# dusk-network/plonk_gadgets

Hardware: AMD Instinct MI355X
Metric: gadget constraints/sec (range_check 256-bit) (higher is better)
Workload: dtype u64x4 (BLS12-381 scalar, Montgomery limbs)

## Files before the change

### plonk_gadgets_amd/csrc/capi_composer.inc

```

struct pg_composer {
    pg_engine *e = nullptr;
    hipStream_t stream = nullptr;
    uint64_t gate_cap = 0, var_cap = 0, n = 0, nvars = 0, zero_var = 0;
    pg::ComposerCols cols{};
    uint64_t *d_stage = nullptr;
    std::vector<uint64_t> pi_gate;
    std::vector<pg_scalar> pi_val;
    std::vector<pg::FourthWire> fourth;
    std::vector<pg::PermSeg> segs;
    void *perm_small = nullptr, *perm_big = nullptr, *val_ws = nullptr;
    void *perm_pieces = nullptr;
    size_t perm_pieces_bytes = 0;
    size_t perm_small_bytes = 0, perm_big_bytes = 0, val_ws_bytes = 0;
    std::vector<void *> ragged;
    uint64_t *h_total = nullptr;
    uint64_t perm_last_sparse = 0;
    uint64_t sparse_hint = 0;
    uint64_t sparse_cap_first = 0;
    bool auto_grow = false;
    uint64_t col_stride = 0;
    void *block = nullptr;
    struct Queued {
        uint8_t kind;
// ... 1245 lines not shown
    add_ragged_segment(c, batch, lay.n_gates, lay.n_vars, 2 * 255 + 5, 255 + 262, b.row_off, b.var_off, 0, pg::WIRES_MAX_BOUND);
    c->n += lay.n_gates;
    c->nvars += lay.n_vars;
    return PG_OK;
}

pg_status pg_composer_is_non_zero_batch(pg_composer *c, const pg_variable *d_var, uint64_t batch, uint8_t *d_err_mask,
                                        uint64_t *err_count) {
    if (!c) return fail(PG_ERR_INVALID_ARGUMENT, "composer is NULL");
    PG_TRY(flush(c));
    if (err_count) *err_count = 0;
    if (batch == 0) return PG_OK;
    PG_TRY(check_u64s(d_var, "d_var"));
    pg_composer::Sig dg;
    PG_TRY(check_var_arrays(c, {d_var}, batch, &dg));
    PG_HIP_TRY(hipSetDevice(c->e->device));
    PG_TRY(perm_reserve(c, &c->val_ws, &c->val_ws_bytes, batch * 32));
    uint4 *vals = static_cast<uint4 *>(c->val_ws);
    const uint64_t want = (2 * batch + pg::kThreads - 1) / pg::kThreads;
    const uint32_t grid = (uint32_t)(want < (uint64_t)c->e->num_cus * 32 ? want : (uint64_t)c->e->num_cus * 32);
    hipLaunchKernelGGL(pg::gather_wire_values_kernel, dim3(grid), dim3(pg::kThreads), 0, c->stream, d_var, c->cols.vars, batch, vals);
    PG_HIP_TRY(hipGetLastError());
    RaggedBuffers b;
    PG_TRY(ragged_alloc(batch, false, &b));
    pg_layout lay;
    uint64_t errs = 0;
    pg_status st = pg_is_non_zero_plan(c->e, reinterpret_cast<const pg_scalar *>(vals), batch, b.row_off, b.var_off, d_err_mask, &lay,
                                       &errs, c->stream);
    const bool failed_items = st == PG_ERR_NON_EXISTING_INVERSE;
    if (failed_items) st = PG_OK;
    if (st == PG_OK) st = need(c, lay.n_gates, lay.n_vars);
    if (st == PG_OK) {
        const pg_columns at = cols_at(c, c->n, c->nvars);
        SignedAppend sa(c, gadget_sig(c, 28, pg::fr_zero(), pg::fr_zero(), batch, errs ? 0x8000000000000000ull | ++c->unmatched : 0, dg),
                        lay.n_gates);
        st = is_non_zero_common(c->e, d_var, reinterpret_cast<const pg_scalar *>(vals), batch, b.row_off, b.var_off, c->n, c->nvars,
                                c->zero_var, &at, c->stream, sa.in_place);
        if (st == PG_OK) sa.commit();
    }
    if (st != PG_OK) {
        (void)hipStreamSynchronize(c->stream);
        b.release();
        return st;
    }
    b.keep(c);
    if (errs == 0)
        add_segment(c, batch, lay.n_gates, lay.n_vars, 2, pg::WIRES_IS_NON_ZERO);
    else
        add_ragged_segment(c, batch, lay.n_gates, lay.n_vars, 3, 3, b.row_off, b.var_off, 2, pg::WIRES_IS_NON_ZERO);
    c->n += lay.n_gates;
    c->nvars += lay.n_vars;
    if (err_count) *err_count = errs;
    return failed_items ? fail(PG_ERR_NON_EXISTING_INVERSE, std::to_string(errs) + " item(s) without an inverse") : PG_OK;
}

pg_status pg_composer_scalar_mix_batch(pg_composer *c, const pg_scalar *d_v, const pg_scalar *d_y, const pg_scalar *d_s,
                                       const pg_scalar *d_a, const pg_scalar *d_b, uint64_t batch, pg_variable *d_result_vars,
                                       uint8_t *d_err_mask, uint64_t *err_count) {
    if (!c) return fail(PG_ERR_INVALID_ARGUMENT, "composer is NULL");
    PG_TRY(flush(c));
    if (err_count) *err_count = 0;
    if (batch == 0) return PG_OK;
    PG_HIP_TRY(hipSetDevice(c->e->device));
    RaggedBuffers b;
    PG_TRY(ragged_alloc(batch, false, &b));
    pg_layout lay;
    uint64_t errs = 0;
    pg_status st = pg_scalar_mix_plan(c->e, d_v, batch, b.row_off, b.var_off, d_err_mask, &lay, &errs, c->stream);
    const bool failed_items = st == PG_ERR_NON_EXISTING_INVERSE;
    if (failed_items) st = PG_OK;
    if (st == PG_OK) st = need(c, lay.n_gates, lay.n_vars);
    if (st == PG_OK) {
        const pg_columns at = cols_at(c, c->n, c->nvars);
        SignedAppend sa(c, gadget_sig(c, 13, pg::fr_zero(), pg::fr_zero(), batch, errs ? 0x8000000000000000ull | ++c->unmatched : 0), lay.n_gates);
        st = scalar_mix_common(c->e, d_v, d_y, d_s, d_a, d_b, batch, b.row_off, b.var_off, c->n, c->nvars, c->zero_var, &at, d_result_vars,
                               c->stream, sa.in_place);
        if (st == PG_OK) sa.commit();
    }
    if (st != PG_OK) {
        (void)hipStreamSynchronize(c->stream);
        b.release();
        return st;
    }
    b.keep(c);
    if (errs == 0)
        add_segment(c, batch, lay.n_gates, lay.n_vars, 0, pg::WIRES_MIX, 0);
    else
        add_ragged_segment(c, batch, lay.n_gates, lay.n_vars, 10, 15, b.row_off, b.var_off, 0, pg::WIRES_MIX);
    c->n += lay.n_gates;
    c->nvars += lay.n_vars;
    if (err_count) *err_count = errs;
    return failed_items ? fail(PG_ERR_NON_EXISTING_INVERSE, std::to_string(errs) + " item(s) without an inverse") : PG_OK;
}

namespace {
pg_status gate_batch(pg_composer *c, uint32_t op, const pg_variable *d_a, const pg_variable *d_b, const pg_variable *d_c,
                     const pg::Fr &q_m, const pg::Fr &q_l, const pg::Fr &q_r, const pg::Fr &q_o, const pg::Fr &q_c, uint64_t batch,
                     pg_variable *d_out_vars) {
    if (!c) return fail(PG_ERR_INVALID_ARGUMENT, "composer is NULL");
    PG_TRY(flush(c));
    if (batch == 0) return PG_OK;
    const bool creates = op == pg::OP_ADD || op == pg::OP_MUL;
    PG_TRY(check_u64s(d_a, "first Variable array"));
    PG_TRY(check_u64s(d_b, "second Variable array"));
    if (!creates) PG_TRY(check_u64s(d_c, "third Variable array"));
    PG_TRY(check_u64s(d_out_vars, "d_out_vars", true));
    for (const pg::Fr *q : {&q_m, &q_l, &q_r, &q_o, &q_c})
        if (!is_reduced(*q)) return fail(PG_ERR_INVALID_ARGUMENT, "selector is not a reduced BlsScalar");
    pg_composer::Sig dg;
    PG_TRY(check_var_arrays(c, {d_a, d_b == d_a ? nullptr : d_b, creates || d_c == d_a ? nullptr : d_c}, batch, &dg));
    PG_TRY(need(c, batch, creates ? batch : 0));
    PG_HIP_TRY(hipSetDevice(c->e->device));
    SigHasher h;
    h.u64(29); h.u64(op); h.u64(batch); h.u64((d_b == d_a ? 1 : 0) | (!creates && d_c == d_a ? 2 : 0) | (!creates && d_c == d_b ? 4 : 0));
    h.fr(q_m); h.fr(q_l); h.fr(q_r); h.fr(q_o); h.fr(q_c); h.u64(dg.a); h.u64(dg.b);
    h.u64(c->n); h.u64(c->nvars); h.u64(c->zero_var);
    SignedAppend sa(c, h.done(), batch);
    pg::GateBatch B{};
    B.op = op | (sa.in_place ? pg::OP_ROW_IN_PLACE : 0u); B.gate0 = c->n; B.var0 = c->nvars; B.batch = batch;
    B.a = d_a; B.b = d_b; B.c = creates ? nullptr : d_c; B.out_vars = d_out_vars;
    B.q_m = q_m; B.q_l = q_l; B.q_r = q_r; B.q_o = q_o; B.q_c = q_c;
    const uint64_t want = (batch + pg::kThreads - 1) / pg::kThreads, most = (uint64_t)c->e->num_cus * 32;
    hipLaunchKernelGGL(pg::gate_batch_kernel, dim3((uint32_t)(want < most ? want : most)), dim3(pg::kThreads), 0, c->stream, B, c->cols);
    PG_HIP_TRY(hipGetLastError());
    sa.commit();
    if (creates || batch >= 4096) add_segment(c, batch, batch, creates ? batch : 0, creates ? 2 : 3, creates ? pg::WIRES_GATE_OUT : pg::WIRES_GATE_ROWS);
    c->n += batch;
    if (creates) c->nvars += batch;
    return PG_OK;
}
}

pg_status pg_composer_poly_gate_batch(pg_composer *c, const pg_variable *d_a, const pg_variable *d_b, const pg_variable *d_c,
                                      const pg_scalar *q_m, const pg_scalar *q_l, const pg_scalar *q_r, const pg_scalar *q_o,
                                      const pg_scalar *q_c, uint64_t batch) {
    if (!q_m || !q_l || !q_r || !q_o || !q_c) return fail(PG_ERR_INVALID_ARGUMENT, "NULL argument");
    return gate_batch(c, pg::OP_ROW, d_a, d_b, d_c, to_fr(q_m), to_fr(q_l), to_fr(q_r), to_fr(q_o), to_fr(q_c), batch, nullptr);
}
pg_status pg_composer_add_batch(pg_composer *c, const pg_scalar *q_l, const pg_variable *d_a, const pg_scalar *q_r,
                                const pg_variable *d_b, const pg_scalar *q_c, uint64_t batch, pg_variable *d_out_vars) {
    if (!q_l || !q_r || !q_c) return fail(PG_ERR_INVALID_ARGUMENT, "NULL argument");
    return gate_batch(c, pg::OP_ADD, d_a, d_b, nullptr, pg::fr_zero(), to_fr(q_l), to_fr(q_r), pg::fr_neg_one(), to_fr(q_c), batch, d_out_vars);
}
pg_status pg_composer_mul_batch(pg_composer *c, const pg_scalar *q_m, const pg_variable *d_a, const pg_variable *d_b,
                                const pg_scalar *q_c, uint64_t batch, pg_variable *d_out_vars) {
    if (!q_m || !q_c) return fail(PG_ERR_INVALID_ARGUMENT, "NULL argument");
    return gate_batch(c, pg::OP_MUL, d_a, d_b, nullptr, to_fr(q_m), pg::fr_zero(), pg::fr_zero(), pg::fr_neg_one(), to_fr(q_c), batch, d_out_vars);
}
pg_status pg_composer_constrain_to_constant_batch(pg_composer *c, const pg_variable *d_a, const pg_scalar *constant, uint64_t batch) {
    if (!constant) return fail(PG_ERR_INVALID_ARGUMENT, "NULL argument");
    return gate_batch(c, pg::OP_ROW, d_a, d_a, d_a, pg::fr_zero(), pg::fr_one(), pg::fr_zero(), pg::fr_zero(), pg::fr_neg(to_fr(constant)),
                      batch, nullptr);
}
pg_status pg_composer_boolean_gate_batch(pg_composer *c, const pg_variable *d_a, uint64_t batch) {
    return gate_batch(c, pg::OP_ROW, d_a, d_a, d_a, pg::fr_one(), pg::fr_zero(), pg::fr_zero(), pg::fr_neg_one(), pg::fr_zero(), batch, nullptr);
}

pg_status pg_composer_add_input_batch(pg_composer *c, const pg_scalar *d_scalars, uint64_t batch, pg_variable *first_var) {
    if (!c || !first_var) return fail(PG_ERR_INVALID_ARGUMENT, "NULL argument");
    PG_TRY(flush(c));
    PG_TRY(need(c, 0, batch));
    if (batch) {
        PG_TRY(check_scalars(d_scalars, "d_scalars"));
        PG_HIP_TRY(hipSetDevice(c->e->device));
        PG_HIP_TRY(hipMemcpyAsync(c->cols.vars + 2 * c->nvars, d_scalars, batch * 32, hipMemcpyDeviceToDevice, c->stream));
    }
    *first_var = c->nvars;
    c->nvars += batch;
    return PG_OK;
}

pg_status pg_composer_copy_out(pg_composer *c, uint64_t gate_first, uint64_t n_gates, uint64_t var_first, uint64_t n_vars,
                               const pg_columns *dst) {
    if (!c || !dst) return fail(PG_ERR_INVALID_ARGUMENT, "NULL argument");
    PG_TRY(flush(c));
    if (gate_first + n_gates > c->n || var_first + n_vars > c->nvars) return fail(PG_ERR_INVALID_ARGUMENT, "range past the end");
    PG_HIP_TRY(hipSetDevice(c->e->device));
    const pg_columns src = cols_at(c, gate_first, var_first);
    pg_scalar *const ds[5] = {dst->q_m, dst->q_l, dst->q_r, dst->q_o, dst->q_c};
    const pg_scalar *const ss[5] = {src.q_m, src.q_l, src.q_r, src.q_o, src.q_c};
    for (int i = 0; i < 5; i++)
        if (ds[i] && n_gates) PG_HIP_TRY(hipMemcpyAsync(ds[i], ss[i], n_gates * 32, hipMemcpyDeviceToDevice, c->stream));
    uint64_t *const dw[3] = {dst->w_l, dst->w_r, dst->w_o};
    const uint64_t *const sw[3] = {src.w_l, src.w_r, src.w_o};
    for (int i = 0; i < 3; i++)
        if (dw[i] && n_gates) PG_HIP_TRY(hipMemcpyAsync(dw[i], sw[i], n_gates * 8, hipMemcpyDeviceToDevice, c->stream));
    if (dst->var_values && n_vars)
        PG_HIP_TRY(hipMemcpyAsync(dst->var_values, src.var_values, n_vars * 32, hipMemcpyDeviceToDevice, c->stream));
    return PG_OK;
}

pg_status pg_composer_read_value(pg_composer *c, pg_variable v, pg_scalar *out) {
    if (!c || !out) return fail(PG_ERR_INVALID_ARGUMENT, "NULL argument");
    PG_TRY(flush(c));
    PG_TRY(check_var(c, v));
    PG_HIP_TRY(hipMemcpyAsync(out, c->cols.vars + 2 * v, 32, hipMemcpyDeviceToHost, c->stream));
    PG_HIP_TRY(hipStreamSynchronize(c->stream));
    return PG_OK;
}

static pg_status upload_sparse(pg_composer *c, CallBuffers &B, uint64_t **d_gate, uint4 **d_val, pg::FourthWire **d_fw) {
    *d_gate = nullptr; *d_val = nullptr; *d_fw = nullptr;
    const size_t np = c->pi_gate.size(), nf = c->fourth.size();
    if (np) {
        PG_HIP_TRY(hipMalloc(d_gate, np * 8));
        B.own(*d_gate);
        PG_HIP_TRY(hipMalloc(d_val, np * 32));
        B.own(*d_val);
        PG_HIP_TRY(hipMemcpyAsync(*d_gate, c->pi_gate.data(), np * 8, hipMemcpyHostToDevice, c->stream));
        PG_HIP_TRY(hipMemcpyAsync(*d_val, c->pi_val.data(), np * 32, hipMemcpyHostToDevice, c->stream));
    }
    if (nf) {
        PG_HIP_TRY(hipMalloc(d_fw, nf * sizeof(pg::FourthWire)));
        B.own(*d_fw);
        PG_HIP_TRY(hipMemcpyAsync(*d_fw, c->fourth.data(), nf * sizeof(pg::FourthWire), hipMemcpyHostToDevice, c->stream));
    }
    return PG_OK;
}

pg_status pg_composer_check(pg_composer *c, int64_t *first_bad) {
    if (!c || !first_bad) return fail(PG_ERR_INVALID_ARGUMENT, "NULL argument");
    PG_TRY(flush(c));
    PG_HIP_TRY(hipSetDevice(c->e->device));
    CallBuffers B(c->stream);
    uint64_t *d_gate; uint4 *d_val; pg::FourthWire *d_fw;
    PG_TRY(upload_sparse(c, B, &d_gate, &d_val, &d_fw));
    unsigned long long *d_bad = nullptr, h_bad = ~0ull;
    PG_HIP_TRY(hipMalloc(&d_bad, 8));
    B.own(d_bad);
    PG_HIP_TRY(hipMemcpyAsync(d_bad, &h_bad, 8, hipMemcpyHostToDevice, c->stream));
    const uint64_t want = (c->n + pg::kThreads - 1) / pg::kThreads;
    const uint32_t grid = (uint32_t)(want < (uint64_t)c->e->num_cus * 8 ? (want ? want : 1) : (uint64_t)c->e->num_cus * 8);
    hipLaunchKernelGGL(pg::check_kernel, dim3(grid), dim3(pg::kThreads), 0, c->stream, c->cols, c->n, (uint64_t)0, c->nvars,
                       c->zero_var, d_gate, d_val, (uint32_t)c->pi_gate.size(), d_fw, (uint32_t)c->fourth.size(), d_bad);
    PG_HIP_TRY(hipGetLastError());
    PG_HIP_TRY(hipMemcpyAsync(&h_bad, d_bad, 8, hipMemcpyDeviceToHost, c->stream));
    PG_HIP_TRY(hipStreamSynchronize(c->stream));
    *first_bad = h_bad == ~0ull ? -1 : (int64_t)h_bad;
    return PG_OK;
}

pg_status pg_composer_dense_pi(pg_composer *c, pg_scalar *d_out) {
    if (!c) return fail(PG_ERR_INVALID_ARGUMENT, "composer is NULL");
    PG_TRY(flush(c));
    PG_TRY(check_scalars(d_out, "d_out"));
    PG_HIP_TRY(hipSetDevice(c->e->device));
    PG_HIP_TRY(hipMemsetAsync(d_out, 0, c->n * 32, c->stream));
    CallBuffers B(c->stream);
    uint64_t *d_gate; uint4 *d_val; pg::FourthWire *d_fw;
    PG_TRY(upload_sparse(c, B, &d_gate, &d_val, &d_fw));
    const uint32_t np = (uint32_t)c->pi_gate.size();
    if (np) {
        hipLaunchKernelGGL(pg::scatter_pi_kernel, dim3((np + 255) / 256), dim3(256), 0, c->stream,
                           reinterpret_cast<uint4 *>(d_out), d_gate, d_val, np);
        PG_HIP_TRY(hipGetLastError());
    }
    PG_HIP_TRY(hipStreamSynchronize(c->stream));
    return PG_OK;
}

pg_status pg_composer_materialize(pg_composer *c, const pg_full_columns *out) {
    if (!c || !out) return fail(PG_ERR_INVALID_ARGUMENT, "NULL argument");
    PG_TRY(flush(c));
    PG_HIP_TRY(hipSetDevice(c->e->device));
    const uint32_t grid = (uint32_t)c->e->num_cus * 32;
    pg::MaterializeOut M{};
    pg_scalar *const consts[7] = {out->q_4, out->q_arith, out->q_range, out->q_logic, out->q_fixed_group_add,
                                  out->q_variable_group_add, out->w_4_value};
    for (int k = 0; k < 7; k++) {
        if (!consts[k]) continue;
        PG_TRY(check_scalars(consts[k], "constant column"));
        M.konst[k] = reinterpret_cast<uint4 *>(consts[k]);
    }
    pg_scalar *const vals[3] = {out->w_l_value, out->w_r_value, out->w_o_value};
    for (int i = 0; i < 3; i++) {
        if (!vals[i]) continue;
        PG_TRY(check_scalars(vals[i], "wire value column"));
        M.val[i] = reinterpret_cast<uint4 *>(vals[i]);
    }
    if (out->w_4) {
        PG_TRY(check_u64s(out->w_4, "w_4"));
        M.w_4 = out->w_4;
    }
    const auto generic = [&](uint64_t lo, uint64_t hi) {
        if (hi <= lo) return;
        const uint64_t want = (2 * (hi - lo) + 16383) / 16384;
        hipLaunchKernelGGL(pg::materialize_kernel, dim3((uint32_t)(want < grid ? want : grid)), dim3(pg::kThreads), 0, c->stream, c->cols, M,
                           lo, hi, c->zero_var);
    };
    uint64_t at = 0;
    for (const pg::PermSeg &s : c->segs) {
        if (s.V > pg::kMatWindowVars || s.V == 0 || s.gate_end - s.gate_base < 4096) continue;
        generic(at, s.gate_base);
        uint64_t group = pg::kMatWindowVars / (s.V ? s.V : 1);
        group = group < 1 ? 1 : (group > s.items ? s.items : group);
#ifndef PG_MAT_GRID_PER_CU
#define PG_MAT_GRID_PER_CU 64
#endif
        const uint64_t n_groups = (s.items + group - 1) / group, most = (uint64_t)c->e->num_cus * PG_MAT_GRID_PER_CU;
        const dim3 mgrid((uint32_t)(n_groups < most ? n_groups : most));
        const bool closed = s.wire_kind != pg::WIRES_UNKNOWN && !s.row_off && (pg::ladder_foreign_per_item(s.wire_kind) == 0 || group <= pg::kMatWitItems);
#define PG_MAT_LAUNCH(MODE, KIND)                                                                                                          \
    hipLaunchKernelGGL((pg::materialize_items_kernel<MODE, KIND>), mgrid, dim3(pg::kMatThreads), 0, c->stream, c->cols, M, s, (uint32_t)group, \
                       c->zero_var)
        if (s.row_off && s.wire_kind == pg::WIRES_MAX_BOUND && group <= pg::kMatWitItems)
            hipLaunchKernelGGL((pg::materialize_items_kernel<pg::MAT_SELF, pg::WIRES_MAX_BOUND, true>), mgrid, dim3(pg::kMatThreads), 0, c->stream,
                               c->cols, M, s, (uint32_t)group, c->zero_var);
        else if (s.row_off && s.wire_kind == pg::WIRES_MIX && group < 127)
            hipLaunchKernelGGL((pg::materialize_items_kernel<pg::MAT_SELF, pg::WIRES_MIX, true>), mgrid, dim3(pg::kMatThreads), 0, c->stream,
                               c->cols, M, s, (uint32_t)group, c->zero_var);
        else if (!closed) PG_MAT_LAUNCH(pg::MAT_READ_WIRES, pg::WIRES_UNKNOWN);
        else if (s.wire_kind == pg::WIRES_RANGE_CHECK) PG_MAT_LAUNCH(pg::MAT_SELF, pg::WIRES_RANGE_CHECK);
        else if (s.wire_kind == pg::WIRES_MAX_BOUND) PG_MAT_LAUNCH(pg::MAT_SELF, pg::WIRES_MAX_BOUND);
        else if (s.wire_kind == pg::WIRES_RANGE_CHECK_ALLOCATED) PG_MAT_LAUNCH(pg::MAT_SELF, pg::WIRES_RANGE_CHECK_ALLOCATED);
        else if (s.wire_kind == pg::WIRES_MAX_BOUND_ALLOCATED) PG_MAT_LAUNCH(pg::MAT_SELF, pg::WIRES_MAX_BOUND_ALLOCATED);
        else if (s.wire_kind == pg::WIRES_DECOMPOSITION) PG_MAT_LAUNCH(pg::MAT_SELF, pg::WIRES_DECOMPOSITION);
        else if (s.wire_kind == pg::WIRES_MIX) PG_MAT_LAUNCH(pg::MAT_SELF, pg::WIRES_MIX);
        else PG_MAT_LAUNCH(pg::MAT_READ_WIRES, pg::WIRES_UNKNOWN);
#undef PG_MAT_LAUNCH
        at = s.gate_end;
    }
    generic(at, c->n);
    CallBuffers B(c->stream);
    uint64_t *d_gate; uint4 *d_val; pg::FourthWire *d_fw;
    PG_TRY(upload_sparse(c, B, &d_gate, &d_val, &d_fw));
    if (d_fw)
        hipLaunchKernelGGL(pg::patch_fourth_kernel, dim3(1), dim3(64), 0, c->stream, reinterpret_cast<uint4 *>(out->q_4), out->w_4,
                           reinterpret_cast<uint4 *>(out->w_4_value), c->cols.vars, d_fw, (uint32_t)c->fourth.size());
    PG_HIP_TRY(hipGetLastError());
    PG_HIP_TRY(hipStreamSynchronize(c->stream));
    return PG_OK;
}

#ifndef PG_PERM_LDS_PAD
#define PG_PERM_LDS_PAD 0
#endif
static pg_status perm_reserve(pg_composer *c, void **buf, size_t *have, size_t bytes) {
    if (bytes <= *have) return PG_OK;
    PG_HIP_TRY(hipStreamSynchronize(c->stream));
    if (*buf) (void)hipFree(*buf);
    *buf = nullptr;
    *have = 0;
    PG_HIP_TRY(hipMalloc(buf, bytes));
    *have = bytes;
    return PG_OK;
}

pg_status pg_composer_permutation_reserve(pg_composer *c, uint64_t sparse_positions) {
    if (!c) return fail(PG_ERR_INVALID_ARGUMENT, "composer is NULL");
    c->sparse_cap_first = sparse_positions;
    if (sparse_positions) c->perm_last_sparse = 0;
    return PG_OK;
}

pg_status pg_composer_permutation(pg_composer *c, uint64_t padded_n, uint64_t *d_sigma) {
    if (!c) return fail(PG_ERR_INVALID_ARGUMENT, "composer is NULL");
    PG_TRY(flush(c));
    PG_TRY(check_u64s(d_sigma, "d_sigma"));
    if (padded_n < c->n) return fail(PG_ERR_INVALID_ARGUMENT, "padded_n is smaller than the circuit");
    PG_HIP_TRY(hipSetDevice(c->e->device));
    const uint32_t grid = (uint32_t)c->e->num_cus * 32;
    if (!c->h_total) PG_HIP_TRY(hipHostMalloc(reinterpret_cast<void **>(&c->h_total), 32, hipHostMallocDefault));
    uint32_t pos_bits = 2, var_bits = 1;
    while ((1ull << pos_bits) < 4 * c->n) pos_bits++;
    while ((1ull << var_bits) < c->nvars + 1) var_bits++;
    if (pos_bits + var_bits > 64) return fail(PG_ERR_INVALID_ARGUMENT, "circuit too large for 64-bit (Variable, position) keys");
    std::vector<pg::PermSeg> segs;
    std::vector<std::pair<uint64_t, uint64_t>> gaps;
    uint64_t at = 0, gap_rows = 0;
    for (pg::PermSeg s : c->segs) {
        const auto fits = [&](uint64_t k) {
            return 4 * k * s.L < pg::kPermDone && k * s.V < pg::kPermNone &&
                   pg::perm_local_lds_bytes((uint32_t)(k * s.L), (uint32_t)(k * s.V)) <= pg::kPermLocalLdsLimit;
        };
        if (!fits(1)) continue;
        uint64_t k = 1024 / s.L;
        k = k < 1 ? 1 : (k > s.items ? s.items : k);
        while (k > 1 && !fits(k)) k--;
        const bool closed_ladder = s.wire_kind != pg::WIRES_UNKNOWN && s.wire_kind < pg::WIRES_MIX && (s.row_off ? s.wire_kind == pg::WIRES_MAX_BOUND && s.tail == 0 : s.wire_n >= 2);
        if (closed_ladder || (pg::is_template_kind(s.wire_kind) && s.tail == 0)) k = 1;
        s.group = (uint32_t)k;
        if (s.gate_base > at) gaps.emplace_back(at, s.gate_base);
        segs.push_back(s);
        at = s.gate_end;
    }
    if (c->n > at) gaps.emplace_back(at, c->n);
    for (const auto &g : gaps) gap_rows += g.second - g.first;
    const size_t seg_bytes = (segs.size() * sizeof(pg::PermSeg) + 255) / 256 * 256;
    const size_t fw_bytes = (c->fourth.size() * sizeof(pg::FourthWire) + 255) / 256 * 256;
    PG_TRY(perm_reserve(c, &c->perm_small, &c->perm_small_bytes, seg_bytes + fw_bytes + 256));
    char *small = static_cast<char *>(c->perm_small);
    pg::PermCtx X;
    X.C = c->cols; X.n = c->n; X.padded_n = padded_n; X.zero_var = c->zero_var;
    X.segs = reinterpret_cast<const pg::PermSeg *>(small); X.n_segs = (uint32_t)segs.size();
    X.fw = reinterpret_cast<const pg::FourthWire *>(small + seg_bytes); X.n_fw = (uint32_t)c->fourth.size();
    X.fw_lo = 0; X.fw_span = 0; X.pos_bits = pos_bits;
    X.hole_key = pos_bits + var_bits >= 64 ? ~0ull : (1ull << (pos_bits + var_bits)) - 1;
    if (!c->fourth.empty()) {
        uint64_t lo = ~0ull, hi = 0;
        for (const pg::FourthWire &f : c->fourth) { lo = f.gate < lo ? f.gate : lo; hi = f.gate > hi ? f.gate : hi; }
        X.fw_lo = lo; X.fw_span = hi - lo;
    }
    uint64_t reserved = 0;
    for (pg::PermSeg &s : segs)
        if (s.wire_kind != pg::WIRES_UNKNOWN && !s.row_off && s.wire_n >= 2) {
            s.sparse_base = reserved;
            reserved += s.items * pg::ladder_foreign_per_item(s.wire_kind);
        } else if (pg::is_template_kind(s.wire_kind) && s.tail == 0) {
            s.sparse_base = reserved;
            reserved += s.items * pg::template_foreign_per_item(s.wire_kind);
        }
    const auto ragged_ladder = [](const pg::PermSeg &s) { return s.row_off && s.wire_kind == pg::WIRES_MAX_BOUND && s.tail == 0; };
    const auto template_seg = [](const pg::PermSeg &s) { return pg::is_template_kind(s.wire_kind) && s.tail == 0; };
    const auto needs_pieces = [&](const pg::PermSeg &s) { return ragged_ladder(s) || (template_seg(s) && s.row_off); };
    const auto pieces_of = [](const pg::PermSeg &s) { return (s.gate_end - (s.gate_base & ~1ull) + pg::kPermLadderRows - 1) / pg::kPermLadderRows; };
    {
        uint64_t total_pieces = 0;
        for (const pg::PermSeg &s : segs)
            if (needs_pieces(s)) total_pieces += pieces_of(s);
        if (total_pieces) {
            PG_TRY(perm_reserve(c, &c->perm_pieces, &c->perm_pieces_bytes, total_pieces * sizeof(uint32_t)));
            uint32_t *at_piece = static_cast<uint32_t *>(c->perm_pieces);
            for (pg::PermSeg &s : segs)
                if (needs_pieces(s)) {
                    s.piece_item = at_piece;
                    at_piece += pieces_of(s);
                    const uint64_t want = (s.items + pg::kThreads - 1) / pg::kThreads;
                    hipLaunchKernelGGL(pg::perm_piece_items_kernel, dim3((uint32_t)(want < grid ? want : grid)), dim3(pg::kThreads), 0, c->stream, s,
                                       pg::kPermLadderRows, at_piece - pieces_of(s));
                }
            PG_HIP_TRY(hipGetLastError());
        }
    }
    unsigned long long *d_count = reinterpret_cast<unsigned long long *>(small + seg_bytes + fw_bytes);
    if (!segs.empty())
        PG_HIP_TRY(hipMemcpyAsync(small, segs.data(), segs.size() * sizeof(pg::PermSeg), hipMemcpyHostToDevice, c->stream));
    if (!c->fourth.empty())
        PG_HIP_TRY(hipMemcpyAsync(small + seg_bytes, c->fourth.data(), c->fourth.size() * sizeof(pg::FourthWire),
                                  hipMemcpyHostToDevice, c->stream));
    uint64_t cap = c->sparse_cap_first ? c->sparse_cap_first : 4 * gap_rows + c->sparse_hint + (1ull << 16), nS = 0;
    if (cap < c->perm_last_sparse) cap = c->perm_last_sparse;
    uint64_t *k0 = nullptr, *k1 = nullptr, holes = 0;
    size_t tmp_bytes = 0;
    for (int attempt = 0;; attempt++) {
        uint64_t *nul = nullptr;
        PG_HIP_TRY(rocprim::radix_sort_keys(nullptr, tmp_bytes, nul, nul, (size_t)cap, 0u, pos_bits + var_bits, c->stream));
        const size_t kb = (cap * 8 + 255) / 256 * 256;
        PG_TRY(perm_reserve(c, &c->perm_big, &c->perm_big_bytes, 2 * kb + tmp_bytes + 256));
        k0 = reinterpret_cast<uint64_t *>(c->perm_big);
        k1 = reinterpret_cast<uint64_t *>(static_cast<char *>(c->perm_big) + kb);
        const pg::PermSparse Q{k0, d_count, cap};
        hipLaunchKernelGGL(pg::perm_count_init_kernel, dim3(1), dim3(1), 0, c->stream, d_count, reserved);
        for (const pg::PermSeg &s : segs) {
            const uint64_t groups = (s.items + s.group - 1) / s.group, most = (uint64_t)c->e->num_cus * 64;
            if (s.wire_kind != pg::WIRES_UNKNOWN && !s.row_off && s.wire_n >= 2) {
                const uint64_t pieces = (s.gate_end - (s.gate_base & ~1ull) + pg::kPermLadderRows - 1) / pg::kPermLadderRows;
                const uint64_t lmost = pg::kPermLadderRows <= 2048 ? 0x7fffffffull : most;
                if (pg::kPermLadderLds)
                    PG_HIP_TRY(hipFuncSetAttribute(reinterpret_cast<const void *>(pg::perm_ladder_kernel<false>), hipFuncAttributeMaxDynamicSharedMemorySize,
                                                   (int)pg::kPermLadderLds));
                const uint32_t lds = pg::ladder_foreign_per_item(s.wire_kind) ? 0u : pg::kPermLadderLds;
                hipLaunchKernelGGL(pg::perm_ladder_kernel<false>, dim3((uint32_t)(pieces < lmost ? pieces : lmost)), dim3(pg::kThreads), lds,
                                   c->stream, X, s, Q, d_sigma);
                continue;
            }
            if (template_seg(s)) {
                const uint64_t pieces = pieces_of(s);
                if (pieces > 0x7fffffffull) return fail(PG_ERR_INVALID_ARGUMENT, "segment too large for one launch");
                const uint32_t lds = pg::template_foreign_per_item(s.wire_kind) ? 0u : pg::kPermLadderLds - 8192;
                const pg::TemplateRows T = pg::template_rows(s.wire_kind);
                if (s.row_off) {
                    PG_HIP_TRY(hipFuncSetAttribute(reinterpret_cast<const void *>(pg::perm_template_kernel<true>),
                                                   hipFuncAttributeMaxDynamicSharedMemorySize, (int)pg::kPermLadderLds));
                    hipLaunchKernelGGL(pg::perm_template_kernel<true>, dim3((uint32_t)pieces), dim3(pg::kThreads), lds, c->stream, X, s, T, Q, d_sigma);
                } else {
                    PG_HIP_TRY(hipFuncSetAttribute(reinterpret_cast<const void *>(pg::perm_template_kernel<false>),
                                                   hipFuncAttributeMaxDynamicSharedMemorySize, (int)pg::kPermLadderLds));
                    hipLaunchKernelGGL(pg::perm_template_kernel<false>, dim3((uint32_t)pieces), dim3(pg::kThreads), lds, c->stream, X, s, T, Q, d_sigma);
                }
                continue;
            }
            if (ragged_ladder(s)) {
                const uint64_t pieces = pieces_of(s);
                if (pieces > 0x7fffffffull) return fail(PG_ERR_INVALID_ARGUMENT, "segment too large for one launch");
                if (pg::kPermLadderLds)
                    PG_HIP_TRY(hipFuncSetAttribute(reinterpret_cast<const void *>(pg::perm_ladder_kernel<true>), hipFuncAttributeMaxDynamicSharedMemorySize,
                                                   (int)pg::kPermLadderLds));
                hipLaunchKernelGGL(pg::perm_ladder_kernel<true>, dim3((uint32_t)pieces), dim3(pg::kThreads), pg::kPermLadderLds, c->stream, X, s, Q,
                                   d_sigma);
                continue;
            }
            hipLaunchKernelGGL(pg::perm_item_kernel, dim3((uint32_t)(groups < most ? groups : most)), dim3(pg::kThreads),
                               pg::perm_local_lds_bytes(s.group * s.L, s.group * s.V) + PG_PERM_LDS_PAD, c->stream, X, s, groups, Q, d_sigma);
        }
        for (const auto &g : gaps) {
            const uint64_t nblk = (g.second - g.first + pg::kPermChunk - 1) / pg::kPermChunk;
            hipLaunchKernelGGL(pg::perm_gap_kernel, dim3((uint32_t)nblk), dim3(pg::kThreads), 0, c->stream, X, g.first, g.second, Q,
                               d_sigma);
        }
        PG_HIP_TRY(hipMemcpyAsync(c->h_total, d_count, 16, hipMemcpyDeviceToHost, c->stream));
        PG_HIP_TRY(hipStreamSynchronize(c->stream));
        nS = c->h_total[0];
        holes = c->h_total[1];
        c->perm_last_sparse = nS;
        if (nS <= cap) break;
        if (attempt) return fail(PG_ERR_HIP, "sparse position list grew between two passes");
        cap = nS;
    }
    if (nS) {
        PG_HIP_TRY(rocprim::radix_sort_keys(static_cast<char *>(c->perm_big) + 2 * ((cap * 8 + 255) / 256 * 256), tmp_bytes, k0, k1,
                                            (size_t)nS, 0u, pos_bits + var_bits, c->stream));
        nS -= holes;
    }
    if (nS) {
        const uint64_t want = (nS + pg::kThreads - 1) / pg::kThreads;
        hipLaunchKernelGGL(pg::perm_sparse_link_kernel, dim3((uint32_t)(want < grid ? want : grid)), dim3(pg::kThreads), 0, c->stream,
                           X, k1, nS, d_sigma);
        if (!segs.empty()) {
            const uint64_t wantw = (nS + 255) / 256;
            hipLaunchKernelGGL(pg::perm_splice_kernel, dim3((uint32_t)(wantw < grid ? wantw : grid)), dim3(pg::kThreads), 0, c->stream,
                               X, k1, nS, d_sigma);
        }
    }
    if (padded_n > c->n) {
        const uint64_t per_run = ((padded_n - c->n) / 2 + 1 + pg::kPermIdentityUnits - 1) / pg::kPermIdentityUnits;
        if (4 * per_run > 0x7fffffffull) return fail(PG_ERR_INVALID_ARGUMENT, "padding too large for one launch");
        PG_HIP_TRY(hipFuncSetAttribute(reinterpret_cast<const void *>(pg::perm_identity_kernel), hipFuncAttributeMaxDynamicSharedMemorySize,
                                       (int)pg::kPermIdentityLds));
        hipLaunchKernelGGL(pg::perm_identity_kernel, dim3((uint32_t)(4 * per_run)), dim3(pg::kThreads), pg::kPermIdentityLds, c->stream,
                           d_sigma, c->n, padded_n);
    }
    PG_HIP_TRY(hipGetLastError());
    return PG_OK;
}

pg_status pg_check_rows(pg_engine *e, const pg_columns *cols, uint64_t n_gates, uint64_t var_base, uint64_t n_vars,
                        pg_variable zero_var, int64_t *first_bad, void *stream) {
    if (!e || !first_bad) return fail(PG_ERR_INVALID_ARGUMENT, "NULL argument");
    *first_bad = -1;
    if (n_gates == 0) return PG_OK;
    PG_TRY(check_columns(cols));
    PG_HIP_TRY(hipSetDevice(e->device));
    hipStream_t st = static_cast<hipStream_t>(stream);
    pg::ComposerCols C;
    C.q[0] = reinterpret_cast<uint4 *>(cols->q_m); C.q[1] = reinterpret_cast<uint4 *>(cols->q_l);
    C.q[2] = reinterpret_cast<uint4 *>(cols->q_r); C.q[3] = reinterpret_cast<uint4 *>(cols->q_o);
    C.q[4] = reinterpret_cast<uint4 *>(cols->q_c);
    C.w[0] = cols->w_l; C.w[1] = cols->w_r; C.w[2] = cols->w_o;
    C.vars = reinterpret_cast<uint4 *>(cols->var_values);
    unsigned long long *d_bad = nullptr, h_bad = ~0ull;
    PG_HIP_TRY(hipMalloc(&d_bad, 8));
    PG_HIP_TRY(hipMemcpyAsync(d_bad, &h_bad, 8, hipMemcpyHostToDevice, st));
    hipLaunchKernelGGL(pg::check_kernel, dim3((uint32_t)e->num_cus * 16), dim3(pg::kThreads), 0, st, C, n_gates, var_base, n_vars,
                       zero_var, (const uint64_t *)nullptr, (const uint4 *)nullptr, 0u, (const pg::FourthWire *)nullptr, 0u, d_bad);
    hipError_t le = hipGetLastError();
    if (le == hipSuccess) le = hipMemcpyAsync(&h_bad, d_bad, 8, hipMemcpyDeviceToHost, st);
    if (le == hipSuccess) le = hipStreamSynchronize(st);
    (void)hipFree(d_bad);
    if (le != hipSuccess) return fail(PG_ERR_HIP, std::string("pg_check_rows: ") + hipGetErrorString(le));
    *first_bad = h_bad == ~0ull ? -1 : (int64_t)h_bad;
    return PG_OK;
}

}
```

### plonk_gadgets_amd/csrc/materialize.hpp

```cpp
#pragma once

#include "permutation.hpp"

namespace pg {

#ifndef PG_MAT_THREADS
#define PG_MAT_THREADS 512
#endif
#ifndef PG_MAT_UNROLL
#define PG_MAT_UNROLL 2
#endif
#ifndef PG_MAT_LOADS
#define PG_MAT_LOADS 8
#endif
constexpr int kMatStoreThreads = PG_MAT_THREADS, kMatThreads = kMatStoreThreads + 64;
constexpr uint32_t kMatWindowVars = 1040;
constexpr uint32_t kMatTailRows = 16;

enum : int {
    MAT_READ_WIRES = 0,
    MAT_SELF = 2,
};
constexpr uint32_t kMatWitItems = 4;

template <int MODE, uint32_t KIND, bool RAGGED = false>
__global__ __launch_bounds__(kMatThreads) void materialize_items_kernel(const ComposerCols C, const MaterializeOut M, const PermSeg S,
                                                                        uint32_t group, uint64_t zero_var) {
    constexpr bool CLOSED = MODE != MAT_READ_WIRES;
    constexpr bool kForeign = KIND == WIRES_RANGE_CHECK_ALLOCATED || KIND == WIRES_MAX_BOUND_ALLOCATED || KIND == WIRES_DECOMPOSITION;
    __shared__ uint4 s_win[2][2 * kMatWindowVars];
    __shared__ uint4 s_tail[2][MODE == MAT_SELF ? kMatTailRows * 6 : 1];
    __shared__ uint4 s_wit[2][MODE == MAT_SELF ? kMatWitItems * 2 : 1];
    constexpr bool BITS = MODE == MAT_SELF && (KIND == WIRES_MAX_BOUND || (!RAGGED && (KIND == WIRES_RANGE_CHECK ||
                                                KIND == WIRES_RANGE_CHECK_ALLOCATED || KIND == WIRES_MAX_BOUND_ALLOCATED)));
    constexpr uint32_t kBlocks = (KIND == WIRES_RANGE_CHECK || KIND == WIRES_RANGE_CHECK_ALLOCATED) ? 2u : 1u;
    constexpr uint32_t kX0 = (KIND == WIRES_RANGE_CHECK || KIND == WIRES_MAX_BOUND) ? 1u : 0u;
    __shared__ uint4 s_tc[2][BITS ? kMatWitItems * 2 * 2 : 1];
    constexpr uint32_t kOff = KIND == WIRES_MIX ? 128 : kMatWitItems + 1;
    __shared__ uint32_t s_off[2][RAGGED ? 2 * kOff : 1];
    __shared__ uint64_t s_base[2][RAGGED ? 2 : 1];
    static_assert(!RAGGED || (MODE == MAT_SELF && (KIND == WIRES_MAX_BOUND || KIND == WIRES_MIX)),
                  "ragged closed forms: max_bound with per-item bounds, the fused mix with items that stopped at their error");
    const uint32_t tid = threadIdx.x;
    const bool loader = tid >= (uint32_t)kMatStoreThreads;
    FrVec one;
    one.f = fr_one();
    const uint4 v1 = (tid & 1) ? one.v[1] : one.v[0], v0 = make_uint4(0, 0, 0, 0);
    const uint64_t n_groups = (S.items + group - 1) / group;
    struct Group { uint64_t r0, r1, w0, ubeg, uend; uint32_t nv, items; };
    const uint32_t foreign_row = KIND == WIRES_DECOMPOSITION ? 2 * S.wire_n + 1
                                 : KIND == WIRES_RANGE_CHECK_ALLOCATED || KIND == WIRES_MAX_BOUND_ALLOCATED ? 0u : kWitnessWire;
    const uint32_t foreign_wire = KIND == WIRES_DECOMPOSITION ? 1u : 0u;
    const uint32_t recip_L = (uint32_t)(((1ull << 32) + S.L - 1) / (S.L ? S.L : 1));
    auto group_of = [&](uint64_t g, int lds_buf) {
        Group G;
        const uint64_t i0 = g * group, i1 = i0 + group < S.items ? i0 + group : S.items;
        G.items = (uint32_t)(i1 - i0);
        if constexpr (RAGGED) {
            if (lds_buf >= 0) {
                G.r0 = S.gate_base + s_base[lds_buf][0];
                G.r1 = G.r0 + s_off[lds_buf][G.items];
                G.w0 = S.var_base + s_base[lds_buf][1];
                G.nv = s_off[lds_buf][kOff + G.items];
            } else {
                G.r0 = S.gate_base + S.row_off[i0];
                G.r1 = S.gate_base + S.row_off[i1];
                G.w0 = S.var_base + S.var_off[i0];
                G.nv = (uint32_t)(S.var_off[i1] - S.var_off[i0]);
            }
        } else if constexpr (CLOSED) {
            G.r0 = S.gate_base + i0 * S.L;
            G.r1 = S.gate_base + i1 * S.L;
            G.w0 = S.var_base + i0 * S.V;
            G.nv = (uint32_t)(i1 - i0) * S.V;
        } else {
            G.r0 = S.gate_base + perm_rows_before(S, i0);
            G.r1 = S.gate_base + perm_rows_before(S, i1);
            G.w0 = S.var_base + perm_vars_before(S, i0);
            G.nv = (uint32_t)(S.var_base + perm_vars_before(S, i1) - G.w0);
        }
        const uint64_t last = 2 * S.gate_end;
        G.ubeg = g == 0 ? 2 * G.r0 : (2 * G.r0 + 31) & ~31ull;
        G.uend = g + 1 == n_groups ? 2 * G.r1 : (2 * G.r1 + 31) & ~31ull;
        G.ubeg = G.ubeg < last ? G.ubeg : last;
        G.uend = G.uend < last ? G.uend : last;
        return G;
    };
    auto fetch = [&](uint64_t g, uint32_t buf) {
        const Group G = group_of(g, -1);
        const uint32_t units = 2 * G.nv, lane = tid - kMatStoreThreads;
        const uint4 *src = C.vars + 2 * G.w0;
        uint4 *win = s_win[buf];
        constexpr uint32_t kRuns = BITS ? kBlocks + 1 : 1;
        const uint32_t n_runs = BITS ? G.items * kRuns : 1;
        const uint32_t VBk = S.wire_n + 261;
#pragma unroll 1
        for (uint32_t run = 0; run < n_runs; run++) {
        uint32_t rb = 0, re = units;
        if constexpr (BITS) {
            const uint32_t it = run / kRuns, r = run - it * kRuns;
            uint32_t vb = it * S.V, Vi = S.V;
            if constexpr (RAGGED) {
                const uint64_t i0 = g * group;
                vb = (uint32_t)(S.var_off[i0 + it] - S.var_off[i0]);
                Vi = (uint32_t)(S.var_off[i0 + it + 1] - S.var_off[i0 + it]);
            }
            rb = 2 * (vb + (r == 0 ? 0 : kX0 + (r - 1) * VBk + 257));
            re = 2 * (vb + (r == kBlocks ? Vi : kX0 + r * VBk + 1));
        }
        uint32_t u = rb + lane;
        const uint32_t units = re;
        for (; u + (PG_MAT_LOADS - 1) * 64 < units; u += PG_MAT_LOADS * 64) {
            const uint4 *q = src + u;
            uint4 *d = win + u;
#if PG_MAT_LOADS >= 8
            const uint4 t0 = q[0], t1 = q[64], t2 = q[128], t3 = q[192], t4 = q[256], t5 = q[320], t6 = q[384], t7 = q[448];
#if PG_MAT_LOADS >= 16
            const uint4 t8 = q[512], t9 = q[576], ta = q[640], tb = q[704], tc = q[768], td = q[832], te = q[896], tf = q[960];
#endif
            d[0] = t0; d[64] = t1; d[128] = t2; d[192] = t3; d[256] = t4; d[320] = t5; d[384] = t6; d[448] = t7;
#if PG_MAT_LOADS >= 16
            d[512] = t8; d[576] = t9; d[640] = ta; d[704] = tb; d[768] = tc; d[832] = td; d[896] = te; d[960] = tf;
#endif
#else
            const uint4 t0 = q[0], t1 = q[64], t2 = q[128], t3 = q[192];
            d[0] = t0; d[64] = t1; d[128] = t2; d[192] = t3;
#endif
        }
        for (; u < units; u += 64) win[u] = src[u];
        }
        if constexpr (BITS) {
            if (lane < G.items * kBlocks) {
                const uint32_t it = lane / kBlocks, b = lane - it * kBlocks;
                uint32_t vb = it * S.V;
                if constexpr (RAGGED) vb = (uint32_t)(S.var_off[g * group + it] - S.var_off[g * group]);
                const uint4 *tp = win + 2 * (vb + kX0 + b * VBk);
                FrVec t;
                t.v[0] = tp[0];
                t.v[1] = tp[1];
                t.f = fr_from_mont(t.f);
                s_tc[buf][2 * lane] = t.v[0];
                s_tc[buf][2 * lane + 1] = t.v[1];
            }
        }
        if constexpr (MODE == MAT_SELF) {
            const uint32_t rows = (uint32_t)((G.uend - 2 * G.r1) >> 1);
            if (lane < 3 * rows) {
                uint32_t rr = lane / 3, vb = 0, n = S.wire_n;
                const uint32_t k = lane - 3 * rr;
                if constexpr (RAGGED) {
                    uint64_t it = g * group + G.items;
                    const uint64_t rows0 = S.row_off[it], vars0 = S.var_off[it];
                    while (S.row_off[it + 1] - rows0 <= rr) it++;
                    const uint64_t first = S.row_off[it];
                    n = KIND == WIRES_MIX ? (S.row_off[it + 1] - first == 10 ? 0u : 1u)
                                          : (uint32_t)(S.row_off[it + 1] - first - 5) >> 1;
                    rr -= (uint32_t)(first - rows0);
                    vb = (uint32_t)(S.var_off[it] - vars0);
                } else {
                    for (; rr >= S.L; rr -= S.L) vb += S.V;
                }
                uint32_t off[3];
                seg_wire_offsets(KIND, n, rr, off, S.tail);
                const uint32_t o = k == 0 ? off[0] : k == 1 ? off[1] : off[2];
                const uint64_t var = o == kWitnessWire ? C.w[k][G.r1 + lane / 3] : o == kZeroWire ? zero_var : G.w0 + G.nv + vb + o;
                s_tail[buf][2 * lane] = C.vars[2 * var];
                s_tail[buf][2 * lane + 1] = C.vars[2 * var + 1];
            }
            if constexpr (RAGGED) {
                const uint64_t i0 = g * group;
                for (uint32_t e = lane; e < kOff; e += 64) {
                    s_off[buf][e] = e <= G.items ? (uint32_t)(S.row_off[i0 + e] - S.row_off[i0]) : 0xffffffffu;
                    s_off[buf][kOff + e] = e <= G.items ? (uint32_t)(S.var_off[i0 + e] - S.var_off[i0]) : 0u;
                }
                if (lane == 47) {
                    s_base[buf][0] = S.row_off[i0];
                    s_base[buf][1] = S.var_off[i0];
                }
            }
            if (foreign_row != kWitnessWire && lane >= 48 && lane - 48 < G.items) {
                const uint64_t var = C.w[foreign_wire][G.r0 + (uint64_t)(lane - 48) * S.L + foreign_row];
                s_wit[buf][2 * (lane - 48)] = C.vars[2 * var];
                s_wit[buf][2 * (lane - 48) + 1] = C.vars[2 * var + 1];
            }
        }
    };
    uint64_t g = blockIdx.x;
    if (loader && g < n_groups) fetch(g, 0);
    __syncthreads();
    for (uint32_t buf = 0; g < n_groups; g += gridDim.x, buf ^= 1) {
        if (loader) {
            if (g + gridDim.x < n_groups) fetch(g + gridDim.x, buf ^ 1);
            lds_barrier();
            continue;
        }
        const uint4 *win = s_win[buf];
        const Group G = group_of(g, (int)buf);
        const uint64_t r0 = G.r0, w0 = G.w0, ubeg = G.ubeg, uend = G.uend;
        const uint32_t nv = G.nv;
        constexpr int U = PG_MAT_UNROLL;
        for (uint64_t ub = (ubeg & ~7ull) + tid; ub < uend; ub += (uint64_t)U * kMatStoreThreads) {
            uint64_t idx[U][3];
            uint4 got[U][3];
#pragma unroll
            for (int j = 0; j < U; j++) {
                const uint64_t u = ub + (uint64_t)j * kMatStoreThreads;
                const uint64_t r = (u < ubeg ? ubeg : (u < uend ? u : uend - 1)) >> 1;
                const uint32_t half = (uint32_t)(u & 1);
                if constexpr (CLOSED) {
                    uint32_t rr = (uint32_t)(r - r0), it, vb, n = S.wire_n;
                    if constexpr (RAGGED) {
                        it = 0;
                        if constexpr (KIND == WIRES_MIX) {
#pragma unroll
                            for (uint32_t step = kOff / 2; step; step >>= 1)
                                if (s_off[buf][it + step] <= rr) it += step;
                        } else {
#pragma unroll
                            for (uint32_t e = 1; e < kMatWitItems; e++) it += rr >= s_off[buf][e] ? 1u : 0u;
                        }
                        const uint32_t first = s_off[buf][it];
                        n = KIND == WIRES_MIX ? (s_off[buf][it + 1] - first == 10 ? 0u : 1u) : (s_off[buf][it + 1] - first - 5) >> 1;
                        vb = s_off[buf][kOff + it];
                        rr -= first;
                    } else {
                        it = __umulhi(rr, recip_L);
                        vb = it * S.V;
                        rr -= it * S.L;
                    }
                    uint32_t off[3];
                    seg_wire_offsets(KIND, n, rr, off, S.tail);
                    {
                        const bool along = r >= G.r1;
                        const uint32_t t = along ? (uint32_t)(r - G.r1) * 6 + half : 0;
#pragma unroll
                        for (int k = 0; k < 3; k++) {
                            const uint32_t rel = vb + off[k];
                            const uint4 *src = win + 2 * (rel < nv ? rel : 0) + half;
                            if constexpr (kForeign)
                                if (off[k] == kWitnessWire) src = s_wit[buf] + 2 * (it < kMatWitItems ? it : 0) + half;
                            if (along) src = s_tail[buf] + t + 2 * k;
                            got[j][k] = *src;
                            if constexpr (BITS) {
                                uint32_t kk = off[k] - kX0, blk = 0;
                                if (kBlocks == 2 && kk >= S.wire_n + 261 && off[k] != kWitnessWire) { kk -= S.wire_n + 261; blk = 1; }
                                if (kk - 1 < 256u && off[k] != kWitnessWire && !along) {
                                    const uint32_t bit = kk - 1, w = bit >> 5;
                                    const uint4 q = s_tc[buf][2 * ((it < kMatWitItems ? it : 0) * kBlocks + blk) + (w >> 2)];
                                    const uint32_t word = (w & 3) == 0 ? q.x : (w & 3) == 1 ? q.y : (w & 3) == 2 ? q.z : q.w;
                                    got[j][k] = (word >> (bit & 31)) & 1u ? v1 : v0;
                                }
                            }
                            if constexpr (KIND == WIRES_MIX)
                                if (off[k] == kZeroWire && !along) got[j][k] = make_uint4(0, 0, 0, 0);
                        }
                    }
                } else {
#pragma unroll
                    for (int k = 0; k < 3; k++) idx[j][k] = M.val[k] ? C.w[k][r] : w0;
                }
            }
            if constexpr (MODE != MAT_SELF) {
#pragma unroll
                for (int j = 0; j < U; j++) {
                    const uint32_t half = (uint32_t)((ub + (uint64_t)j * kMatStoreThreads) & 1);
#pragma unroll
                    for (int k = 0; k < 3; k++) {
                        const uint64_t rel = idx[j][k] - w0;
                        got[j][k] = rel < nv ? win[2 * (uint32_t)rel + half] : C.vars[2 * idx[j][k] + half];
                    }
                }
            }
#pragma unroll
            for (int j = 0; j < U; j++) {
                const uint64_t u = ub + (uint64_t)j * kMatStoreThreads;
                if (u >= ubeg && u < uend) {
#pragma unroll
                    for (int k = 0; k < 7; k++)
                        if (M.konst[k]) store16(M.konst[k] + u, k == 1 ? v1 : v0);
                    if (M.w_4 && !(u & 1)) M.w_4[u >> 1] = zero_var;
#pragma unroll
                    for (int k = 0; k < 3; k++)
                        if (M.val[k]) store16(M.val[k] + u, got[j][k]);
                }
            }
        }
        lds_barrier();
    }
}

}
```

Before: 32.57 billion.

## Recompute bit-decomposition accumulators in loader wave instead of copying window vars

For bit-decomposition segments, the loader wave no longer copies the whole variable window from global memory. It loads only a few data vars per item, then derives the bit and accumulator values from the constant with a wave-level prefix scan over a shared table of powers of two. Tail rows get the same treatment. The loader loop is also reorganised so the loader wave runs its own fetch loop and barrier sequence instead of branching inside the store loop. This trades global memory reads for field additions in a single 64-lane wave, and the reworked barrier pairing between loader and store threads is a correctness risk.

```diff
diff --git a/plonk_gadgets_amd/csrc/capi_composer.inc b/plonk_gadgets_amd/csrc/capi_composer.inc
--- a/plonk_gadgets_amd/csrc/capi_composer.inc
+++ b/plonk_gadgets_amd/csrc/capi_composer.inc
@@ -1571,13 +1571,13 @@
         const bool closed = s.wire_kind != pg::WIRES_UNKNOWN && !s.row_off && (pg::ladder_foreign_per_item(s.wire_kind) == 0 || group <= pg::kMatWitItems);
 #define PG_MAT_LAUNCH(MODE, KIND)                                                                                                          \
     hipLaunchKernelGGL((pg::materialize_items_kernel<MODE, KIND>), mgrid, dim3(pg::kMatThreads), 0, c->stream, c->cols, M, s, (uint32_t)group, \
-                       c->zero_var)
+                       c->zero_var, c->e->d_pow2)
         if (s.row_off && s.wire_kind == pg::WIRES_MAX_BOUND && group <= pg::kMatWitItems)
             hipLaunchKernelGGL((pg::materialize_items_kernel<pg::MAT_SELF, pg::WIRES_MAX_BOUND, true>), mgrid, dim3(pg::kMatThreads), 0, c->stream,
-                               c->cols, M, s, (uint32_t)group, c->zero_var);
+                               c->cols, M, s, (uint32_t)group, c->zero_var, c->e->d_pow2);
         else if (s.row_off && s.wire_kind == pg::WIRES_MIX && group < 127)
             hipLaunchKernelGGL((pg::materialize_items_kernel<pg::MAT_SELF, pg::WIRES_MIX, true>), mgrid, dim3(pg::kMatThreads), 0, c->stream,
-                               c->cols, M, s, (uint32_t)group, c->zero_var);
+                               c->cols, M, s, (uint32_t)group, c->zero_var, c->e->d_pow2);
         else if (!closed) PG_MAT_LAUNCH(pg::MAT_READ_WIRES, pg::WIRES_UNKNOWN);
         else if (s.wire_kind == pg::WIRES_RANGE_CHECK) PG_MAT_LAUNCH(pg::MAT_SELF, pg::WIRES_RANGE_CHECK);
         else if (s.wire_kind == pg::WIRES_MAX_BOUND) PG_MAT_LAUNCH(pg::MAT_SELF, pg::WIRES_MAX_BOUND);
diff --git a/plonk_gadgets_amd/csrc/materialize.hpp b/plonk_gadgets_amd/csrc/materialize.hpp
--- a/plonk_gadgets_amd/csrc/materialize.hpp
+++ b/plonk_gadgets_amd/csrc/materialize.hpp
@@ -21,11 +21,16 @@
     MAT_READ_WIRES = 0,
     MAT_SELF = 2,
 };
+__device__ __forceinline__ bool mat_bit(const Fr &c, uint32_t i) {
+    const uint32_t w = i >> 6;
+    const uint64_t x = w == 0 ? c.l[0] : w == 1 ? c.l[1] : w == 2 ? c.l[2] : c.l[3];
+    return (x >> (i & 63)) & 1u;
+}
 constexpr uint32_t kMatWitItems = 4;
 
 template <int MODE, uint32_t KIND, bool RAGGED = false>
 __global__ __launch_bounds__(kMatThreads) void materialize_items_kernel(const ComposerCols C, const MaterializeOut M, const PermSeg S,
-                                                                        uint32_t group, uint64_t zero_var) {
+                                                                        uint32_t group, uint64_t zero_var, const uint4 *pow2) {
     constexpr bool CLOSED = MODE != MAT_READ_WIRES;
     constexpr bool kForeign = KIND == WIRES_RANGE_CHECK_ALLOCATED || KIND == WIRES_MAX_BOUND_ALLOCATED || KIND == WIRES_DECOMPOSITION;
     __shared__ uint4 s_win[2][2 * kMatWindowVars];
@@ -36,6 +41,8 @@
     constexpr uint32_t kBlocks = (KIND == WIRES_RANGE_CHECK || KIND == WIRES_RANGE_CHECK_ALLOCATED) ? 2u : 1u;
     constexpr uint32_t kX0 = (KIND == WIRES_RANGE_CHECK || KIND == WIRES_MAX_BOUND) ? 1u : 0u;
     __shared__ uint4 s_tc[2][BITS ? kMatWitItems * 2 * 2 : 1];
+    __shared__ uint4 s_pow[BITS ? 2 * 256 : 1];
+    constexpr uint32_t kData = kX0 + 1 + (kBlocks == 2 ? 8 : 3);
     constexpr uint32_t kOff = KIND == WIRES_MIX ? 128 : kMatWitItems + 1;
     __shared__ uint32_t s_off[2][RAGGED ? 2 * kOff : 1];
     __shared__ uint64_t s_base[2][RAGGED ? 2 : 1];
@@ -91,25 +98,8 @@
         const uint32_t units = 2 * G.nv, lane = tid - kMatStoreThreads;
         const uint4 *src = C.vars + 2 * G.w0;
         uint4 *win = s_win[buf];
-        constexpr uint32_t kRuns = BITS ? kBlocks + 1 : 1;
-        const uint32_t n_runs = BITS ? G.items * kRuns : 1;
-        const uint32_t VBk = S.wire_n + 261;
-#pragma unroll 1
-        for (uint32_t run = 0; run < n_runs; run++) {
-        uint32_t rb = 0, re = units;
-        if constexpr (BITS) {
-            const uint32_t it = run / kRuns, r = run - it * kRuns;
-            uint32_t vb = it * S.V, Vi = S.V;
-            if constexpr (RAGGED) {
-                const uint64_t i0 = g * group;
-                vb = (uint32_t)(S.var_off[i0 + it] - S.var_off[i0]);
-                Vi = (uint32_t)(S.var_off[i0 + it + 1] - S.var_off[i0 + it]);
-            }
-            rb = 2 * (vb + (r == 0 ? 0 : kX0 + (r - 1) * VBk + 257));
-            re = 2 * (vb + (r == kBlocks ? Vi : kX0 + r * VBk + 1));
-        }
-        uint32_t u = rb + lane;
-        const uint32_t units = re;
+        if constexpr (!BITS) {
+        uint32_t u = lane;
         for (; u + (PG_MAT_LOADS - 1) * 64 < units; u += PG_MAT_LOADS * 64) {
             const uint4 *q = src + u;
             uint4 *d = win + u;
@@ -128,19 +118,83 @@
 #endif
         }
         for (; u < units; u += 64) win[u] = src[u];
-        }
-        if constexpr (BITS) {
-            if (lane < G.items * kBlocks) {
-                const uint32_t it = lane / kBlocks, b = lane - it * kBlocks;
-                uint32_t vb = it * S.V;
-                if constexpr (RAGGED) vb = (uint32_t)(S.var_off[g * group + it] - S.var_off[g * group]);
-                const uint4 *tp = win + 2 * (vb + kX0 + b * VBk);
-                FrVec t;
-                t.v[0] = tp[0];
-                t.v[1] = tp[1];
-                t.f = fr_from_mont(t.f);
-                s_tc[buf][2 * lane] = t.v[0];
-                s_tc[buf][2 * lane + 1] = t.v[1];
+        } else {
+            auto place = [&](uint32_t it, uint32_t &n) {
+                n = S.wire_n;
+                if constexpr (RAGGED) {
+                    const uint64_t i0 = g * group, v0 = S.var_off[i0 + it];
+                    n = (uint32_t)(S.var_off[i0 + it + 1] - v0) - kX0 - 261;
+                    return (uint32_t)(v0 - S.var_off[i0]);
+                } else {
+                    return it * S.V;
+                }
+            };
+            for (uint32_t e = lane; e < G.items * kData * 2; e += 64) {
+                const uint32_t it = e / (2 * kData), d = (e - it * 2 * kData) >> 1;
+                uint32_t n;
+                const uint32_t vb = place(it, n);
+                uint32_t o = d;
+                if (d > kX0) {
+                    const uint32_t dd = d - (kX0 + 1), blk = kBlocks == 2 ? dd >> 2 : 0;
+                    o = kX0 + blk * (n + 261) + 258 + n + (dd - 4 * blk);
+                }
+                const uint32_t u = 2 * (vb + o) + (e & 1);
+                win[u] = src[u];
+            }
+            const uint32_t nb = G.items * kBlocks, lpb = nb == 1 ? 64 : nb == 2 ? 32 : nb == 3 ? 21 : 16;
+            const uint32_t blkid = nb == 1 ? 0 : nb == 2 ? lane >> 5 : nb == 3 ? lane / 21 : lane >> 4, sub = lane - blkid * lpb;
+            const bool mine = blkid < nb;
+            const uint32_t it = mine ? blkid / kBlocks : 0, b = mine ? blkid - it * kBlocks : 0;
+            uint32_t n;
+            const uint32_t vb = place(it, n);
+            uint4 *tp = win + 2 * (vb + kX0 + b * (n + 261));
+            FrVec t;
+            t.v[0] = tp[0];
+            t.v[1] = tp[1];
+            t.f = fr_from_mont(t.f);
+            if (mine && sub == 0) {
+                s_tc[buf][2 * blkid] = t.v[0];
+                s_tc[buf][2 * blkid + 1] = t.v[1];
+            }
+            const uint32_t per = ((n + lpb) / lpb) | 1u;
+            const uint32_t i0 = sub * per < n + 1 ? sub * per : n + 1;
+            const uint32_t i1 = !mine ? i0 : i0 + per < n + 1 ? i0 + per : n + 1;
+            auto step = [&](const Fr &acc, uint32_t j) {
+                const Fr sum = fr_add(acc, lds_fr(s_pow, j));
+                const bool set = mat_bit(t.f, j);
+                Fr o;
+#pragma unroll
+                for (int l = 0; l < 4; l++) o.l[l] = set ? sum.l[l] : acc.l[l];
+                return o;
+            };
+            Fr run = fr_zero();
+#pragma unroll 1
+            for (uint32_t j = i0; j < i1; j++) run = step(run, j);
+#pragma unroll 1
+            for (uint32_t d = 1; d < 64; d <<= 1) {
+                Fr up;
+#pragma unroll
+                for (int l = 0; l < 4; l++) {
+                    const uint32_t lo = __shfl_up((uint32_t)run.l[l], d), hi = __shfl_up((uint32_t)(run.l[l] >> 32), d);
+                    up.l[l] = (uint64_t)hi << 32 | lo;
+                }
+                const Fr sum = fr_add(run, up);
+                const bool take = sub >= d;
+#pragma unroll
+                for (int l = 0; l < 4; l++) run.l[l] = take ? sum.l[l] : run.l[l];
+            }
+            Fr acc;
+#pragma unroll
+            for (int l = 0; l < 4; l++) {
+                const uint32_t lo = __shfl_up((uint32_t)run.l[l], 1), hi = __shfl_up((uint32_t)(run.l[l] >> 32), 1);
+                acc.l[l] = sub ? (uint64_t)hi << 32 | lo : 0;
+            }
+            uint4 *slot = tp + 2 * 257;
+#pragma unroll 1
+            for (uint32_t i = i0; i < i1; i++) {
+                slot[2 * i] = make_uint4((uint32_t)acc.l[0], (uint32_t)(acc.l[0] >> 32), (uint32_t)acc.l[1], (uint32_t)(acc.l[1] >> 32));
+                slot[2 * i + 1] = make_uint4((uint32_t)acc.l[2], (uint32_t)(acc.l[2] >> 32), (uint32_t)acc.l[3], (uint32_t)(acc.l[3] >> 32));
+                acc = step(acc, i);
             }
         }
         if constexpr (MODE == MAT_SELF) {
@@ -163,9 +217,41 @@
                 uint32_t off[3];
                 seg_wire_offsets(KIND, n, rr, off, S.tail);
                 const uint32_t o = k == 0 ? off[0] : k == 1 ? off[1] : off[2];
-                const uint64_t var = o == kWitnessWire ? C.w[k][G.r1 + lane / 3] : o == kZeroWire ? zero_var : G.w0 + G.nv + vb + o;
-                s_tail[buf][2 * lane] = C.vars[2 * var];
-                s_tail[buf][2 * lane + 1] = C.vars[2 * var + 1];
+                uint64_t var = o == kWitnessWire ? C.w[k][G.r1 + lane / 3] : o == kZeroWire ? zero_var : G.w0 + G.nv + vb + o;
+                uint32_t made = 0, mi = 0;
+                if constexpr (BITS) {
+                    if (o >= kX0 && o != kWitnessWire && o != kZeroWire) {
+                        uint32_t kk = o - kX0, blk = 0;
+                        if (kBlocks == 2 && kk >= n + 261) { kk -= n + 261; blk = 1; }
+                        if (kk - 1 < 257 + n) {
+                            made = kk <= 256 ? 1 : 2;
+                            mi = kk <= 256 ? kk - 1 : kk - 257;
+                            var = G.w0 + G.nv + vb + kX0 + blk * (n + 261);
+                        }
+                    }
+                }
+                uint4 t0 = C.vars[2 * var], t1 = C.vars[2 * var + 1];
+                if constexpr (BITS) {
+                    FrVec t;
+                    t.v[0] = t0;
+                    t.v[1] = t1;
+                    const Fr tc = fr_from_mont(t.f);
+                    Fr acc = fr_zero();
+#pragma unroll 1
+                    for (uint32_t j = 0; j < (made == 2 ? mi : 0u); j++) {
+                        const Fr sum = fr_add(acc, lds_fr(s_pow, j));
+                        const bool set = mat_bit(tc, j);
+#pragma unroll
+                        for (int l = 0; l < 4; l++) acc.l[l] = set ? sum.l[l] : acc.l[l];
+                    }
+                    if (made == 1 && mat_bit(tc, mi)) acc = fr_one();
+                    if (made) {
+                        t0 = make_uint4((uint32_t)acc.l[0], (uint32_t)(acc.l[0] >> 32), (uint32_t)acc.l[1], (uint32_t)(acc.l[1] >> 32));
+                        t1 = make_uint4((uint32_t)acc.l[2], (uint32_t)(acc.l[2] >> 32), (uint32_t)acc.l[3], (uint32_t)(acc.l[3] >> 32));
+                    }
+                }
+                s_tail[buf][2 * lane] = t0;
+                s_tail[buf][2 * lane + 1] = t1;
             }
             if constexpr (RAGGED) {
                 const uint64_t i0 = g * group;
@@ -186,14 +272,19 @@
         }
     };
     uint64_t g = blockIdx.x;
-    if (loader && g < n_groups) fetch(g, 0);
-    __syncthreads();
+    if (loader) {
+        if constexpr (BITS)
+            for (uint32_t u = tid - kMatStoreThreads; u < 2 * 256; u += 64) s_pow[u] = pow2[u];
+#pragma unroll 1
+        for (uint32_t buf = 0;; g += gridDim.x, buf ^= 1) {
+            const bool more = g < n_groups;
+            if (more) fetch(g, buf);
+            lds_barrier();
+            if (!more) return;
+        }
+    }
+    lds_barrier();
     for (uint32_t buf = 0; g < n_groups; g += gridDim.x, buf ^= 1) {
-        if (loader) {
-            if (g + gridDim.x < n_groups) fetch(g + gridDim.x, buf ^ 1);
-            lds_barrier();
-            continue;
-        }
         const uint4 *win = s_win[buf];
         const Group G = group_of(g, (int)buf);
         const uint64_t r0 = G.r0, w0 = G.w0, ubeg = G.ubeg, uend = G.uend;
```

Result: no change. 32.39 billion (-0.6%).
